# biscuitzb/COEB-SLAM

Measured on AMD Instinct MI355X. Metric: frames/sec ORB extract+match @640x480/1000 kp; 1/2/4/8 GPU + %HBM roofline, higher is better.
Workload: dtype u8; 1 GPU; 640x480, 8-level pyramid, 1000 kp, extract + Hamming match to prev frame (BASELINE configs[1]); width=640, height=480, nfeatures=1000, nlevels=8, halo_frames_per_rank=1, pipelines_per_gpu=3, streams_per_gpu=1, ranks=single, parallelism=frame-sharded x1 (no collectives), hw_queues=4, side_stream=own, side_stream_created=with the context

## Files before the change

coeb-slam_amd/csrc/coeb_extract.hip:

```cpp
#include <type_traits>
#include <cmath>
#include <hip/hip_runtime.h>

#include "coeb_internal.hpp"

namespace {

constexpr int kThreads = 256;
constexpr int kWaves = kThreads / 64;

__device__ __forceinline__ int lane_id() { return __lane_id(); }
__device__ __forceinline__ int wave_id() { return __builtin_amdgcn_readfirstlane(threadIdx.x >> 6); }
__device__ __forceinline__ void wave_sync_lds()
{
    __builtin_amdgcn_fence(__ATOMIC_RELEASE, "wavefront");
    __builtin_amdgcn_wave_barrier();
    __builtin_amdgcn_fence(__ATOMIC_ACQUIRE, "wavefront");
}
typedef unsigned int u32x4 __attribute__((ext_vector_type(4)));

__device__ __forceinline__ uint64_t lanemask_lt() { return (1ull << lane_id()) - 1ull; }

__device__ __forceinline__ int wave_sum(int v)
{
// ... 1565 lines not shown
            }
        } else {
            const int G = oct_team<NT>(nd, (K - (n - nd) + nd - 1) / nd);
            divide_nodes(G, S, nd, 0);
        }
        obar();
        int T = 0, nexp = 0;
        for (int base = 0; base < nd; base += NT) {
            const int j = base + tid;
            int e = 0, x = 0;
            if (j < nd) {
                const int4 q = s_cnt[j];
                e = (q.x > 0) + (q.y > 0) + (q.z > 0) + (q.w > 0);
                x = (q.x > 1) + (q.y > 1) + (q.z > 1) + (q.w > 1);
            }
            int tot, tot2;
            const int pre = block_scan_excl<NW>(e, &tot, sbuf);
            block_scan_excl<NW>(x, &tot2, sbuf);
            if (j < nd) s_base[j] = T + pre;
            T += tot;
            nexp += tot2;
        }
        obar();
        const int nnew = T + (n - nd);
        if (nnew > g.ncap) { if (tid == 0) atomicOr(b.err, 4); finish = true; break; }
        for (int j = tid; j < nd; j += NT) {
            const int k = s_work[j];
            const int4 q = s_cnt[j];
            const int s = S.start[k], bf = S.buf[k];
            const int4 r = S.rect[k];
            int a = s_base[j];
            int off = s;
            const int qq[4] = {q.x, q.y, q.z, q.w};
            for (int c4 = 0; c4 < 4; c4++) {
                if (qq[c4] > 0) {
                    const int pos = T - 1 - a;
                    int4 cr; int sx, sy;
                    child_rect(r, c4, &cr, &sx, &sy);
                    D.start[pos] = off; D.cnt[pos] = qq[c4]; D.alloc[pos] = alloc_ctr + a;
                    D.buf[pos] = bf ^ 1; D.rect[pos] = cr;
                    a++;
                }
                off += qq[c4];
            }
        }
        {
            int carry = 0;
            for (int base = 0; base < n; base += NT) {
                const int k = base + tid;
                const bool keep = k < n && S.cnt[k] <= 1;
                int tot;
                const int pre = block_scan_flag<NW>(keep, &tot, sbuf);
                if (keep) {
                    const int pos = T + carry + pre;
                    D.start[pos] = S.start[k]; D.cnt[pos] = S.cnt[k]; D.alloc[pos] = S.alloc[k];
                    D.buf[pos] = S.buf[k]; D.rect[pos] = S.rect[k];
                }
                carry += tot;
            }
        }
        obar();
        alloc_ctr += T;
        n = nnew;
        cs ^= 1;
        if (n >= N || n == prevSize) { finish = true; break; }
        if (n + nexp * 3 > N) { final_phase = true; break; }
    }

    while (final_phase && !finish) {
        const int prevSize = n;
        if (n > OCT_LMAX) { if (tid == 0) atomicOr(b.err, 4); break; }
        NodeRef S = nref(O, cs), D = nref(O, cs ^ 1);
        int m = 0;
        for (int base = 0; base < n; base += NT) {
            const int k = base + tid;
            const bool dv = k < n && S.cnt[k] > 1;
            int tot;
            const int pre = block_scan_flag<NW>(dv, &tot, sbuf);
            if (dv) s_work[m + pre] = k;
            m += tot;
        }
        for (int k = tid; k < n; k += NT) s_dead[k] = 0;
        obar();
        const int avg = m > 0 ? (K - (n - m) + m - 1) / m : 0;
        if (m > 0) divide_nodes(oct_team<NT>(m, avg), S, m, 1);
        for (int j = tid; j < m; j += NT) {
            const int k = s_work[j];
            s_push[j] = (int)(((uint32_t)S.cnt[k] << 16) | (uint32_t)S.alloc[k]);
        }
        obar();
        if (K < 32768 && alloc_ctr < 65536) {
            for (int j = tid; j < m; j += NT) {
                const int kj = s_push[j];
                int rank = 0;
#pragma unroll 8
                for (int i = 0; i < m; i++) rank += s_push[i] > kj;
                s_rank[j] = rank;
            }
        } else {
            for (int j = tid; j < m; j += NT) {
                const int k = s_work[j];
                const int cj = S.cnt[k], aj = S.alloc[k];
                int rank = 0;
                for (int i = 0; i < m; i++) {
                    const int ki = s_work[i];
                    const int ci = S.cnt[ki], ai = S.alloc[ki];
                    rank += (ci > cj) || (ci == cj && ai > aj);
                }
                s_rank[j] = rank;
            }
        }
        obar();
        for (int j = tid; j < m; j += NT) s_base[s_rank[j]] = j;
        obar();
        int nproc = m;
        {
            int carry = 0, found = 0x7fffffff;
            for (int base = 0; base < m; base += NT) {
                const int r = base + tid;
                int d = 0;
                if (r < m) {
                    const int4 q = s_cnt[s_base[r]];
                    d = (q.x > 0) + (q.y > 0) + (q.z > 0) + (q.w > 0) - 1;
                }
                int tot;
                const int pre = block_scan_excl<NW>(d, &tot, sbuf);
                if (r < m && n + carry + pre + d >= N) found = min(found, r);
                carry += tot;
            }
            int fr = found;
            for (int o = 32; o > 0; o >>= 1) fr = min(fr, __shfl_xor(fr, o, 64));
            if (lane == 0) sbuf[wv] = fr;
            obar();
            int mn = 0x7fffffff;
            for (int i = 0; i < NW; i++) mn = min(mn, sbuf[i]);
            obar();
            if (mn != 0x7fffffff) nproc = mn + 1;
        }
        int T = 0;
        for (int base = 0; base < nproc; base += NT) {
            const int r = base + tid;
            int e = 0;
            if (r < nproc) {
                const int4 q = s_cnt[s_base[r]];
                e = (q.x > 0) + (q.y > 0) + (q.z > 0) + (q.w > 0);
            }
            int tot;
            const int pre = block_scan_excl<NW>(e, &tot, sbuf);
            if (r < nproc) s_push[r] = T + pre;
            T += tot;
        }
        for (int j = tid; j < m; j += NT)
            if (s_rank[j] < nproc) s_dead[s_work[j]] = 1;
        obar();
        const int nnew = T + n - nproc;
        if (nnew > g.ncap) { if (tid == 0) atomicOr(b.err, 4); break; }
        divide_nodes(oct_team<NT>(nproc, avg), S, nproc, 2);
        for (int r = tid; r < nproc; r += NT) {
            const int j = s_base[r];
            const int k = s_work[j];
            const int s = S.start[k], bf = S.buf[k];
            const int4 pr = S.rect[k];
            const int4 qc = s_cnt[j];
            {
                int a = s_push[r];
                int off = s;
                const int qq[4] = {qc.x, qc.y, qc.z, qc.w};
                for (int c4 = 0; c4 < 4; c4++) {
                    if (qq[c4] > 0) {
                        const int pos = T - 1 - a;
                        int4 cr; int ssx, ssy;
                        child_rect(pr, c4, &cr, &ssx, &ssy);
                        D.start[pos] = off; D.cnt[pos] = qq[c4]; D.alloc[pos] = alloc_ctr + a;
                        D.buf[pos] = bf ^ 1; D.rect[pos] = cr;
                        a++;
                    }
                    off += qq[c4];
                }
            }
        }
        {
            int carry = 0;
            for (int base = 0; base < n; base += NT) {
                const int k = base + tid;
                const bool keep = k < n && !s_dead[k];
                int tot;
                const int pre = block_scan_flag<NW>(keep, &tot, sbuf);
                if (keep) {
                    const int pos = T + carry + pre;
                    D.start[pos] = S.start[k]; D.cnt[pos] = S.cnt[k]; D.alloc[pos] = S.alloc[k];
                    D.buf[pos] = S.buf[k]; D.rect[pos] = S.rect[k];
                }
                carry += tot;
            }
        }
        obar();
        alloc_ctr += T;
        n = nnew;
        cs ^= 1;
        if (n >= N || n == prevSize) finish = true;
    }
    if (COEB_OCT_CLOCK) oc_t2 = (long long)clock64();

    NodeRef S = nref(O, cs);
    uint32_t* out = b.lvl_kp + (int64_t)f * P->lvl_stride + g.out_off;
    const bool cull = !area && l < 8;
    const float scale = (l != 0) ? g.scale : 1.0f;
    int carry = 0;
    for (int base = 0; base < n; base += NT) {
        const int k = base + tid;
        uint32_t best = 0;
        bool keep = false;
        if (k < n) {
            const uint32_t* src = KB(S.buf[k]) + S.start[k];
            const int c = S.cnt[k];
            best = src[0];
            int maxr = key_s(best);
            for (int q = 1; q < c; q++) {
                const uint32_t kk = src[q];
                if (key_s(kk) > maxr) { best = kk; maxr = key_s(kk); }
            }
            const int x = key_x(best) + 16, y = key_y(best) + 16;
            best = pack_key(x, y, key_s(best));
            keep = !(cull && masked_out(dm, (float)x, (float)y, scale, P->W, P->H));
        }
        int tot;
        const int pre = block_scan_flag<NW>(keep, &tot, sbuf);
        if (keep) {
            if (carry + pre < g.out_cap) out[carry + pre] = best;
            else atomicOr(b.err, 8);
        }
        carry += tot;
    }
    if (tid == 0) b.lvl_n[(int64_t)f * P->L + l] = min(carry, g.out_cap);
    if (COEB_OCT_CLOCK && tid == 0) {
        const int wg = blockIdx.x + gridDim.x * blockIdx.y;
        if (wg < 4096) {
            long long* r = g_oct_clk + 6 * wg;
            r[0] = l; r[1] = K; r[2] = oc_w0;
            r[3] = (long long)clock64() - oc_t0; r[4] = oc_t1 - oc_t0; r[5] = oc_t2 - oc_t1;
        }
    }
}

__device__ float fast_atan2_dev(float y, float x)
{
    const float p1 = 0.9997878412794807f * (float)(180 / 3.1415926535897932384626433832795);
    const float p3 = -0.3258083974640975f * (float)(180 / 3.1415926535897932384626433832795);
    const float p5 = 0.1555786518463281f * (float)(180 / 3.1415926535897932384626433832795);
    const float p7 = -0.04432655554792128f * (float)(180 / 3.1415926535897932384626433832795);
    const float ax = fabsf(x), ay = fabsf(y);
    float a, c, c2;
    if (ax >= ay) {
        c = ay / (ax + (float)2.2204460492503131e-16);
        c2 = c * c;
        a = (((p7 * c2 + p5) * c2 + p3) * c2 + p1) * c;
    } else {
        c = ax / (ay + (float)2.2204460492503131e-16);
        c2 = c * c;
        a = 90.f - (((p7 * c2 + p5) * c2 + p3) * c2 + p1) * c;
    }
    if (x < 0) a = 180.f - a;
    if (y < 0) a = 360.f - a;
    return a;
}

__device__ void sincos_canon(float af, float* s, float* c)
{
    const double two_over_pi = 6.36619772367581382433e-01;
    const double pio2_1 = 1.57079632673412561417e+00;
    const double pio2_1t = 6.07710050650619224932e-11;
    const double S1 = -1.66666666666666324348e-01, S2 = 8.33333333332248946124e-03,
                 S3 = -1.98412698298579493134e-04, S4 = 2.75573137070700676789e-06,
                 S5 = -2.50507602534068634195e-08, S6 = 1.58969099521155010221e-10;
    const double C1 = 4.16666666666666019037e-02, C2 = -1.38888888888741095749e-03,
                 C3 = 2.48015872894767294178e-05, C4 = -2.75573143513906633035e-07,
                 C5 = 2.08757232129817482790e-09, C6 = -1.13596475577881948265e-11;
    const double x = (double)af;
    const double kd = rint(x * two_over_pi);
    double r = __builtin_fma(-kd, pio2_1, x);
    r = __builtin_fma(-kd, pio2_1t, r);
    const double z = r * r;
    const double v = z * r;
    const double sr = S2 + z * (S3 + z * (S4 + z * (S5 + z * S6)));
    const double sn = r + v * (S1 + z * sr);
    const double cr = z * (C1 + z * (C2 + z * (C3 + z * (C4 + z * (C5 + z * C6)))));
    const double hz = 0.5 * z;
    const double w = 1.0 - hz;
    const double cs = w + (((1.0 - w) - hz) + z * cr);
    const int q = ((int)kd) & 3;
    double so, co;
    if (q == 0) { so = sn; co = cs; }
    else if (q == 1) { so = cs; co = -sn; }
    else if (q == 2) { so = -sn; co = -cs; }
    else { so = -cs; co = sn; }
    *s = (float)so;
    *c = (float)co;
}

struct KeyPointOut { float x, y, size, angle, response; int octave, class_id; };

constexpr int kBlRow = 72, kBlRows = 37;
constexpr int kDescGroup = 2;
constexpr int kDescIcBatch = 32;
#ifndef COEB_DESC_KP
#define COEB_DESC_KP 8
#endif
template <int KP> constexpr int desc_slab() { return kBlRow * kBlRows * kDescGroup + 32 * KP; }
constexpr int kUmax[16] = {15, 15, 15, 15, 14, 14, 14, 13, 13, 12, 11, 10, 9, 8, 6, 3};

__device__ __forceinline__ uint32_t ic_mask(int av, int d)
{
    uint32_t w = 0;
    for (int i = 0; i < 4; i++) {
        const int u = 4 * d + i - 15;
        if (av < 16 && (u < 0 ? -u : u) <= kUmax[av]) w |= 0xFFu << (8 * i);
    }
    return w;
}

__device__ __forceinline__ uint32_t dpp_or_xor1(uint32_t v)
{
    return v | (uint32_t)__builtin_amdgcn_mov_dpp((int)v, 0xB1, 0xf, 0xf, false);
}
__device__ __forceinline__ uint32_t dpp_or_xor2(uint32_t v)
{
    return v | (uint32_t)__builtin_amdgcn_mov_dpp((int)v, 0x4E, 0xf, 0xf, false);
}
__device__ __forceinline__ uint32_t dpp_or_shl4(uint32_t v)
{
    return v | (uint32_t)__builtin_amdgcn_mov_dpp((int)v, 0x104, 0xf, 0xf, false);
}

template <bool kVec>
__device__ __forceinline__ void ic_row_load(const uint8_t* rp, uint4& c0, uint4& c1, uint4& c2)
{
    if (kVec) {
        c0 = reinterpret_cast<const uint4*>(rp)[0];
        c1 = reinterpret_cast<const uint4*>(rp)[1];
        c2 = reinterpret_cast<const uint4*>(rp)[2];
    } else {
        uint32_t q[12];
#pragma unroll
        for (int k = 0; k < 12; k++)
            q[k] = (uint32_t)rp[4 * k] | ((uint32_t)rp[4 * k + 1] << 8) | ((uint32_t)rp[4 * k + 2] << 16) |
                   ((uint32_t)rp[4 * k + 3] << 24);
        c0 = make_uint4(q[0], q[1], q[2], q[3]);
        c1 = make_uint4(q[4], q[5], q[6], q[7]);
        c2 = make_uint4(q[8], q[9], q[10], q[11]);
    }
}

template <bool kVec0, int KP>
__global__ __launch_bounds__(kThreads) void k_describe(const Plan* __restrict__ P, ExtractBufs b)
{
    constexpr int kLpk = 64 / KP;
    constexpr int kHl = kLpk / 2;
    constexpr int kNr = 16 / kHl;
    constexpr int kNb = kNr < 4 ? kNr : 4;
    static_assert(KP >= 2 && KP <= 32 && (KP & (KP - 1)) == 0, "KP: power of two in [2, 32]");
    __shared__ __attribute__((aligned(16))) uint8_t s_slab[kWaves][desc_slab<KP>()];
    __shared__ __attribute__((aligned(16))) uint32_t s_msk[17][8];
    if (threadIdx.x < 17 * 8) s_msk[threadIdx.x >> 3][threadIdx.x & 7] = ic_mask(threadIdx.x >> 3, threadIdx.x & 7);
    __syncthreads();
    const int2 bxy = block_xy();
    const int f = bxy.y;
    const int L = P->L;
    const int lane = lane_id(), wv = wave_id();
    const int nl = lane < L ? b.lvl_n[(int64_t)f * L + lane] : 0;
    int incl = nl;
    for (int o = 1; o < COEB_MAXL; o <<= 1) {
        const int y = __shfl_up(incl, o, 64);
        if (lane >= o) incl += y;
    }
    const int total = __builtin_amdgcn_readlane(incl, L - 1);
    if (bxy.x == 0 && threadIdx.x == 0) b.counts[f] = total;
    const int idx0 = (bxy.x * kWaves + wv) * KP;
    if (idx0 >= total) return;
    const int nk = min(KP, total - idx0);
    const int kq = lane / kLpk, half = (lane / kHl) & 1, qi = lane % kHl;
    const int id = idx0 + min(kq, nk - 1);
    int l = 0, start = 0;
    for (int q = 0; q < L - 1; q++) {
        const int e = __builtin_amdgcn_readlane(incl, q);
        if (id >= e) { l = q + 1; start = e; }
    }
    const LevelGeom& g = P->lv[l];
    const uint32_t key = b.lvl_kp[(int64_t)f * P->lvl_stride + g.out_off + (id - start)];
    const int x = key_x(key), y = key_y(key), sc = key_s(key);
    const uint8_t* img = level_ptr(P, b, f, l);
    uint32_t A = 0, S = 0;
    int m01 = 0;
    const int a = (x - 15) & 15;
    const uint32_t m8 = (a & 8) ? 0xFFFFFFFFu : 0u, m4 = (a & 4) ? 0xFFFFFFFFu : 0u;
    const uint8_t* rowp = img + (int64_t)y * g.pitch + (x - 15 - a);
    const int64_t spitch = half ? (int64_t)g.pitch : -(int64_t)g.pitch;
    const bool vec = kVec0 || l != 0;
    int aoff = 15;
    if (vec) {
        constexpr int kTasks = (93 + kLpk - 1) / kLpk;
        constexpr int kBatch = kDescIcBatch < kTasks ? kDescIcBatch : kTasks;
        constexpr uint64_t kUmaxPk = 0x3689ABCDDEEEFFFFull;
        const int j = lane % kLpk;
        const uint8_t* base0 = img + (int64_t)(y - 15) * g.pitch + (x - 15 - a);
#pragma unroll
        for (int i0 = 0; i0 < kTasks; i0 += kBatch) {
        uint4 cq[kBatch];
#pragma unroll
        for (int ii = 0; ii < kBatch; ii++) {
            const int i = i0 + ii;
            if (i >= kTasks) break;
            const int r = min(j + kLpk * i, 92);
            const int row = r / 3, ch = r - 3 * row;
            cq[ii] = *reinterpret_cast<const uint4*>(base0 + (int64_t)row * g.pitch + 16 * ch);
        }
#pragma unroll
        for (int ii = 0; ii < kBatch; ii++) {
            const int i = i0 + ii;
            if (i >= kTasks) break;
            const int r = j + kLpk * i;
            if (r < 93) {
                const int row = r / 3, ch = r - 3 * row;
                const int v = row - 15, av = v < 0 ? -v : v;
                const int um = (int)((kUmaxPk >> (4 * av)) & 15u);
                const uint32_t q[4] = {cq[ii].x, cq[ii].y, cq[ii].z, cq[ii].w};
                uint32_t rs = 0;
#pragma unroll
                for (int d = 0; d < 4; d++) {
                    const int u0 = 16 * ch + 4 * d - a - 15;
                    const int s0 = min(max(-um - u0, 0), 4), e0 = min(max(um - u0 + 1, 0), 4);
                    const uint32_t msk = (uint32_t)((1ull << (8 * e0)) - 1ull) & ~(uint32_t)((1ull << (8 * s0)) - 1ull);
                    const uint32_t pm = q[d] & msk;
                    A = __builtin_amdgcn_udot4(pm, (uint32_t)(u0 + 31) * 0x01010101u + 0x03020100u, A, false);
                    rs = __builtin_amdgcn_udot4(pm, 0x01010101u, rs, false);
                }
                S += rs;
                m01 += v * (int)rs;
            }
        }
        }
        aoff = 31;
    } else {
#pragma unroll
    for (int i0 = 0; i0 < kNr; i0 += kNb) {
        uint4 c[kNb][3];
#pragma unroll
        for (int r = 0; r < kNb; r++) {
            const uint8_t* rp = rowp + (qi + kHl * (i0 + r)) * spitch;
            if (vec) ic_row_load<true>(rp, c[r][0], c[r][1], c[r][2]);
            else ic_row_load<false>(rp, c[r][0], c[r][1], c[r][2]);
        }
#pragma unroll
        for (int r = 0; r < kNb; r++) {
            const int av = qi + kHl * (i0 + r);
            const uint32_t* msk = s_msk[(av == 0 && half) ? 16 : av];
            const uint32_t q[12] = {c[r][0].x, c[r][0].y, c[r][0].z, c[r][0].w, c[r][1].x, c[r][1].y,
                                    c[r][1].z, c[r][1].w, c[r][2].x, c[r][2].y, c[r][2].z, c[r][2].w};
            uint32_t r1[10], r2[9];
#pragma unroll
            for (int k = 0; k < 10; k++) r1[k] = (m8 & q[k + 2]) | (~m8 & q[k]);
#pragma unroll
            for (int k = 0; k < 9; k++) r2[k] = (m4 & r1[k + 1]) | (~m4 & r1[k]);
            uint32_t rs = 0;
#pragma unroll
            for (int d = 0; d < 8; d++) {
                const uint32_t pm = __builtin_amdgcn_alignbyte(r2[d + 1], r2[d], (uint32_t)(a & 3)) & msk[d];
                A = __builtin_amdgcn_udot4(pm, 0x03020100u + 0x04040404u * (uint32_t)d, A, false);
                rs = __builtin_amdgcn_udot4(pm, 0x01010101u, rs, false);
            }
            S += rs;
            m01 += av * (int)rs;
        }
    }
        if (half == 0) m01 = -m01;
    }
#pragma unroll
    for (int o = 1; o < kLpk; o <<= 1) {
        A += __shfl_xor(A, o, 64);
        S += __shfl_xor(S, o, 64);
        m01 += __shfl_xor(m01, o, 64);
    }
    const int m10 = (int)A - aoff * (int)S;
    const float angle = fast_atan2_dev((float)m01, (float)m10);
    const float factorPI = (float)(3.1415926535897932384626433832795 / 180.f);
    float bs, ac;
    sincos_canon(angle * factorPI, &bs, &ac);
    if (lane % kLpk == 0 && kq < nk) {
        float fx = (float)x, fy = (float)y;
        if (l != 0) { fx *= g.scale; fy *= g.scale; }
        KeyPointOut o;
        o.x = fx; o.y = fy; o.size = (float)g.size_i; o.angle = angle; o.response = (float)sc;
        o.octave = l; o.class_id = -1;
        reinterpret_cast<KeyPointOut*>(b.kps)[(int64_t)f * P->kcap + idx0 + kq] = o;
    }
    const int4 pa = reinterpret_cast<const int4*>(b.pattern)[lane];
    float px0[4], py0[4], px1[4], py1[4];
#pragma unroll
    for (int t = 0; t < 4; t++) {
        const int pw = t == 0 ? pa.x : t == 1 ? pa.y : t == 2 ? pa.z : pa.w;
        px0[t] = (float)(int8_t)(pw & 0xff); py0[t] = (float)(int8_t)((pw >> 8) & 0xff);
        px1[t] = (float)(int8_t)((pw >> 16) & 0xff); py1[t] = (float)(int8_t)(pw >> 24);
    }
    uint8_t* slab = s_slab[wv];
    uint32_t* dsl = reinterpret_cast<uint32_t*>(slab + kBlRow * kBlRows * kDescGroup);
    const int xoff = x - ((x - 18) & ~15);
    const uint8_t* blur_f = b.blur + (int64_t)f * P->blur_stride;
    static_assert(kDescGroup == 2, "staging below is written for 2 patches per step");
    uint4 qa0, qa1, qa2, qb0, qb1, qb2;
    const int ty0 = (y - 18) >> 3, dy = (y - 18) & 7, tymax = ((y + 18) >> 3) - ty0;
    const int porg = (int)g.blur_off + (int)blur_tile_off((x - 18) & ~15, ty0 * 8, g.bpitch);
    const int trs = g.bpitch * 8;
    const int lo = ((lane >> 3) & 3) * 128 + (lane & 7) * 16;
    const int tr0 = lane >> 5;
#define COEB_LOAD_PATCH(t, q0, q1, q2)                                                          \
    {                                                                                           \
        const int tt_ = min((t), nk - 1);                                                       \
        const uint8_t* o_ = blur_f + __builtin_amdgcn_readlane(porg, tt_ * kLpk) + lo;          \
        const int trs_ = __builtin_amdgcn_readlane(trs, tt_ * kLpk);                            \
        const int tm_ = __builtin_amdgcn_readlane(tymax, tt_ * kLpk);                           \
        q0 = *reinterpret_cast<const uint4*>(o_ + min(tr0, tm_) * trs_);                        \
        q1 = *reinterpret_cast<const uint4*>(o_ + min(tr0 + 2, tm_) * trs_);                    \
        q2 = *reinterpret_cast<const uint4*>(o_ + min(tr0 + 4, tm_) * trs_);                    \
    }
    COEB_LOAD_PATCH(0, qa0, qa1, qa2)
    COEB_LOAD_PATCH(1, qb0, qb1, qb2)
    for (int t0 = 0; t0 < nk; t0 += kDescGroup) {
        {
            auto put = [&](uint8_t* base, int row, int c, uint4 v) {
                uint2* d = reinterpret_cast<uint2*>(base + row * kBlRow + 16 * c);
                d[0] = make_uint2(v.x, v.y);
                d[1] = make_uint2(v.z, v.w);
            };
            uint8_t* pb = slab + kBlRow * kBlRows;
            const int dya = __builtin_amdgcn_readlane(dy, min(t0, nk - 1) * kLpk);
            const int dyb = __builtin_amdgcn_readlane(dy, min(t0 + 1, nk - 1) * kLpk);
            const int c = (lane >> 3) & 3, r = 8 * tr0 + (lane & 7);
            auto put_t = [&](uint8_t* base, int row, uint4 v) {
                if ((unsigned)row < (unsigned)kBlRows) put(base, row, c, v);
            };
            put_t(slab, r - dya, qa0);
            put_t(slab, r + 16 - dya, qa1);
            put_t(slab, r + 32 - dya, qa2);
            put_t(pb, r - dyb, qb0);
            put_t(pb, r + 16 - dyb, qb1);
            put_t(pb, r + 32 - dyb, qb2);
        }
        wave_sync_lds();
        if (t0 + kDescGroup < nk) {
            COEB_LOAD_PATCH(t0 + 2, qa0, qa1, qa2)
            COEB_LOAD_PATCH(t0 + 3, qb0, qb1, qb2)
        }
#pragma unroll
        for (int k = 0; k < kDescGroup; k++) {
            const int t = t0 + k;
            if (t >= nk) break;
            const float tb = __int_as_float(__builtin_amdgcn_readlane(__float_as_int(bs), t * kLpk));
            const float ta = __int_as_float(__builtin_amdgcn_readlane(__float_as_int(ac), t * kLpk));
            const uint8_t* bc = slab + k * kBlRow * kBlRows + 18 * kBlRow + __builtin_amdgcn_readlane(xoff, t * kLpk);
            const f32x2 AB = {ta, tb}, BA = {tb, ta};
            uint32_t nib = 0;
#pragma unroll
            for (int tt = 0; tt < 4; tt++) {
                const f32x2 t0 = f32x2{py0[tt], py0[tt]} * AB, t1 = f32x2{py1[tt], py1[tt]} * AB;
                const f32x2 rc0 = __builtin_elementwise_fma(f32x2{px0[tt], px0[tt]}, BA, f32x2{t0.x, -t0.y});
                const f32x2 rc1 = __builtin_elementwise_fma(f32x2{px1[tt], px1[tt]}, BA, f32x2{t1.x, -t1.y});
                const int o0 = (int)__builtin_fmaf(rintf(rc0.x), (float)kBlRow, rintf(rc0.y));
                const int o1 = (int)__builtin_fmaf(rintf(rc1.x), (float)kBlRow, rintf(rc1.y));
                nib |= (uint32_t)(bc[o0] < bc[o1]) << tt;
            }
            uint32_t dw = nib << (4 * (lane & 7));
            dw = dpp_or_shl4(dpp_or_xor2(dpp_or_xor1(dw)));
            if ((lane & 7) == 0) dsl[8 * t + (lane >> 3)] = dw;
        }
        wave_sync_lds();
    }
#undef COEB_LOAD_PATCH
    uint4* gd = reinterpret_cast<uint4*>(b.desc + ((int64_t)f * P->kcap + idx0) * 32);
    if (lane < 2 * nk) gd[lane] = reinterpret_cast<const uint4*>(dsl)[lane];
}

}

int fast_timing_read(unsigned long long* out)
{
    static unsigned long long h[256 * 8];
    if (hipMemcpyFromSymbol(h, HIP_SYMBOL(g_fast_clk), sizeof(h)) != hipSuccess) return -1;
    for (int k = 0; k < 8; k++) {
        out[k] = 0;
        for (int i = 0; i < 256; i++) out[k] += h[i * 8 + k];
    }
    static const unsigned long long z[256 * 8] = {};
    return hipMemcpyToSymbol(HIP_SYMBOL(g_fast_clk), z, sizeof(z)) == hipSuccess ? 0 : -1;
}

int oct_timing_read(long long* out)
{
    return hipMemcpyFromSymbol(out, HIP_SYMBOL(g_oct_clk), sizeof(long long) * 4096 * 6) == hipSuccess ? 0 : -1;
}

int launch_extract(const Plan& plan, const Plan* d_plan, const ExtractBufs& b, int F, hipStream_t s,
                   ProfileHook* prof, const SideStream* side)
{
    prof_begin(prof, "k_dynmask", s);
    hipLaunchKernelGGL(k_dynmask, dim3((F + 63) / 64), dim3(64), 0, s, b, F, plan.W, plan.H);
    prof_end(prof, s);
    BlurWork bw;
    bw.L = plan.L;
    int items = 0;
    const int brows = 32;
    static_assert(brows % 8 == 0, "bands start on tile rows");
    bw.brows = brows;
    for (int l = 0; l < plan.L; l++) {
        const LevelGeom& g = plan.lv[l];
        bw.nstrips[l] = (g.w + kBlurCols - 1) / kBlurCols;
        bw.item_off[l] = items;
        bw.nquads[l] = (bw.nstrips[l] + 3) / 4;
        bw.bh[l] = 0;
        items += bw.nquads[l] * ((g.h + brows - 1) / brows);
    }
    bw.item_off[plan.L] = items;
    const char* pb = coeb_switch("COEB_PYR_BYTES");
    const bool pyr_bytes = pb && atoi(pb) != 0;
    const char* frb = coeb_switch("COEB_FAST_RB");
    const int fast_rbytes = frb && atoi(frb) == kFastRowBytes ? kFastRowBytes : fast_rb(plan);
    const int fast_lds = kWaves * fast_wave_lds(plan, fast_rbytes);
    constexpr int kFastPerBlock = kWaves;
    auto blur = [&](hipStream_t st, int i0, int i1) {
        if (i1 <= i0) return;
        BlurWork w = bw;
        w.item0 = i0; w.item1 = i1;
        prof_begin(prof, "k_blur", st);
        hipLaunchKernelGGL(k_blur_rows, dim3((i1 - i0 + kWaves - 1) / kWaves, F), dim3(kThreads), 0,
                           st, d_plan, b, w);
        prof_end(prof, st);
    };
    auto fast = [&](hipStream_t st, int l0, int l1) {
        l1 = std::min(l1, plan.L);
        if (l1 <= l0) return;
        prof_begin(prof, "k_fast", st);
        const int c0 = plan.lv[l0].cell0, c1 = l1 < plan.L ? plan.lv[l1].cell0 : plan.ncells;
        hipLaunchKernelGGL(fast_rbytes == kFastRowBytesM ? k_fast<kFastRowBytesM> : k_fast<kFastRowBytes>,
                           dim3((c1 - c0 + kFastPerBlock - 1) / kFastPerBlock, F), dim3(kThreads), fast_lds,
                           st, d_plan, b, b.cells, c0, c1);
        prof_end(prof, st);
    };
    const bool split = side && side->s && plan.L > 1;
    const int m = split ? 2 : 0;
    if (split) {
        (void)hipEventRecord(side->fork, s);
        (void)hipStreamWaitEvent(side->s, side->fork, 0);
        blur(side->s, 0, bw.item_off[1]);
        fast(side->s, 0, 1);
    }
    for (int l = 1; l < plan.L; l++) {
        const LevelGeom& g = plan.lv[l];
        const LevelGeom& gp = plan.lv[l - 1];
        const uint8_t* src = l == 1 ? b.gray : b.pyr + gp.pyr_off;
        const int64_t src_fs = l == 1 ? (int64_t)plan.W * plan.H : plan.pyr_stride;
        prof_begin(prof, "k_pyr_level", s);
        const bool rows = g.rows_ok && ((gp.pitch | (int)(src_fs & 3) | (int)((uintptr_t)src & 3)) & 3) == 0;
        if (rows && !pyr_bytes) {
            hipLaunchKernelGGL(k_pyr_rows, dim3((g.w + PR_COLS - 1) / PR_COLS, (g.h + kWaves * PR_ROWS - 1) / (kWaves * PR_ROWS), F),
                               dim3(kThreads), 0, s, src, src_fs, gp.pitch, gp.h, b.pyr + g.pyr_off, plan.pyr_stride,
                               g.pitch, g.w, g.h, b.rtab + g.rtab_off, g.xmax, resize_simd_end(g.w),
                               reinterpret_cast<const int4*>(b.rtab + g.yrow_off), b.rtab + g.band_off);
        } else {
            int tsw, tsh;
            pyr_tile_lds(gp.w, gp.h, g.w, g.h, &tsw, &tsh);
            hipLaunchKernelGGL(k_pyr_level, dim3((g.w + PT_W - 1) / PT_W, (g.h + PT_H - 1) / PT_H, F), dim3(kThreads),
                               tsw * tsh, s, src, src_fs, gp.pitch, gp.w, gp.h, b.pyr + g.pyr_off, plan.pyr_stride,
                               g.pitch, g.w, g.h, b.rtab + g.rtab_off, g.xmax, resize_simd_end(g.w), tsw, tsh);
        }
        prof_end(prof, s);
        if (split && l == m - 1) {
            (void)hipEventRecord(side->mid, s);
            (void)hipStreamWaitEvent(side->s, side->mid, 0);
            blur(side->s, bw.item_off[1], bw.item_off[m]);
            fast(side->s, 1, m);
        }
    }
    constexpr int kOctThreads = 256;
    int oct_kl, oct_lds;
    oct_launch_keys(plan, F, &oct_kl, &oct_lds);
    lds_limit_max((const void*)k_octree<kOctThreads>);
    auto octree = [&](hipStream_t st, int l0, int l1) {
        if (l1 <= l0) return;
        prof_begin(prof, "k_octree", st);
        hipLaunchKernelGGL(k_octree<kOctThreads>, dim3(F, l1 - l0), dim3(kOctThreads), oct_lds, st, d_plan, b, l0, plan.oct_w,
                           oct_kl);
        prof_end(prof, st);
    };
    if (split) {
        (void)hipEventRecord(side->pyr_done, s);
        (void)hipStreamWaitEvent(side->s, side->pyr_done, 0);
        blur(side->s, bw.item_off[m], items);
        (void)hipEventRecord(side->join, side->s);
    } else {
        blur(s, 0, items);
    }
    fast(s, m, plan.L);
    if (split) (void)hipStreamWaitEvent(s, side->join, 0);
    octree(s, 0, plan.L);
    prof_begin(prof, "k_describe", s);
    const bool vec0 = plan.W % 16 == 0 && (reinterpret_cast<uintptr_t>(b.gray) & 15) == 0;
    constexpr int KP = COEB_DESC_KP;
    if (vec0)
        hipLaunchKernelGGL((k_describe<true, KP>), dim3((plan.kcap + kWaves * KP - 1) / (kWaves * KP), F), dim3(kThreads), 0,
                           s, d_plan, b);
    else
        hipLaunchKernelGGL((k_describe<false, KP>), dim3((plan.kcap + kWaves * KP - 1) / (kWaves * KP), F), dim3(kThreads), 0,
                           s, d_plan, b);
    prof_end(prof, s);
    return hipGetLastError() == hipSuccess ? 0 : -1;
}
```

Before: 390,800 frames/s.

## Rewrite ORB intensity-centroid path with branchless circle masks and strided row pointers

Reworks the vectorized intensity-centroid moment loop. Instead of computing per-dword min/max byte masks for every row, it precomputes packed umax words at compile time and builds the circular-window mask via byte-wise add/bitop3 tricks, so each dword needs one mask plus two dot4 ops. Row addresses are advanced by a fixed stride per task, and all loads are issued before any compute. It also makes the patch-to-LDS stores branchless by sending out-of-range rows to a dummy LDS area, and skips the LDS mask table init and barrier in the vec-only variant. The cost is more LDS per wave, KP restricted to 8 or 16, and more registers held by the full load batch.

```diff
diff --git a/coeb-slam_amd/csrc/coeb_extract.hip b/coeb-slam_amd/csrc/coeb_extract.hip
--- a/coeb-slam_amd/csrc/coeb_extract.hip
+++ b/coeb-slam_amd/csrc/coeb_extract.hip
@@ -1891,11 +1891,11 @@
 
 constexpr int kBlRow = 72, kBlRows = 37;
 constexpr int kDescGroup = 2;
-constexpr int kDescIcBatch = 32;
+constexpr int kDescDummy = 80;
 #ifndef COEB_DESC_KP
 #define COEB_DESC_KP 8
 #endif
-template <int KP> constexpr int desc_slab() { return kBlRow * kBlRows * kDescGroup + 32 * KP; }
+template <int KP> constexpr int desc_slab() { return kBlRow * kBlRows * kDescGroup + 32 * KP + kDescDummy; }
 constexpr int kUmax[16] = {15, 15, 15, 15, 14, 14, 14, 13, 13, 12, 11, 10, 9, 8, 6, 3};
 
 __device__ __forceinline__ uint32_t ic_mask(int av, int d)
@@ -1907,6 +1907,19 @@
     }
     return w;
 }
+
+template <int kStep, int kN>
+struct IcUmWords {
+    uint32_t w[kN];
+    constexpr IcUmWords() : w{}
+    {
+        for (int m = 0; m < kN; m++)
+            for (int i = 0; i < 8; i++) {
+                const int row = kStep * m + i, v = row - 15;
+                if (row <= 30) w[m] |= (uint32_t)kUmax[v < 0 ? -v : v] << (4 * i);
+            }
+    }
+};
 
 __device__ __forceinline__ uint32_t dpp_or_xor1(uint32_t v)
 {
@@ -1947,11 +1960,13 @@
     constexpr int kHl = kLpk / 2;
     constexpr int kNr = 16 / kHl;
     constexpr int kNb = kNr < 4 ? kNr : 4;
-    static_assert(KP >= 2 && KP <= 32 && (KP & (KP - 1)) == 0, "KP: power of two in [2, 32]");
+    static_assert(KP == 8 || KP == 16, "KP: 8 or 16");
     __shared__ __attribute__((aligned(16))) uint8_t s_slab[kWaves][desc_slab<KP>()];
-    __shared__ __attribute__((aligned(16))) uint32_t s_msk[17][8];
-    if (threadIdx.x < 17 * 8) s_msk[threadIdx.x >> 3][threadIdx.x & 7] = ic_mask(threadIdx.x >> 3, threadIdx.x & 7);
-    __syncthreads();
+    __shared__ __attribute__((aligned(16))) uint32_t s_msk[kVec0 ? 1 : 17][8];
+    if constexpr (!kVec0) {
+        if (threadIdx.x < 17 * 8) s_msk[threadIdx.x >> 3][threadIdx.x & 7] = ic_mask(threadIdx.x >> 3, threadIdx.x & 7);
+        __syncthreads();
+    }
     const int2 bxy = block_xy();
     const int f = bxy.y;
     const int L = P->L;
@@ -1988,45 +2003,46 @@
     int aoff = 15;
     if (vec) {
         constexpr int kTasks = (93 + kLpk - 1) / kLpk;
-        constexpr int kBatch = kDescIcBatch < kTasks ? kDescIcBatch : kTasks;
-        constexpr uint64_t kUmaxPk = 0x3689ABCDDEEEFFFFull;
+        constexpr IcUmWords<kLpk, (kTasks + 2) / 3> kUm;
+        constexpr uint32_t hb = 0x80808080u;
         const int j = lane % kLpk;
-        const uint8_t* base0 = img + (int64_t)(y - 15) * g.pitch + (x - 15 - a);
-#pragma unroll
-        for (int i0 = 0; i0 < kTasks; i0 += kBatch) {
-        uint4 cq[kBatch];
-#pragma unroll
-        for (int ii = 0; ii < kBatch; ii++) {
-            const int i = i0 + ii;
-            if (i >= kTasks) break;
-            const int r = min(j + kLpk * i, 92);
+        const uint8_t* base0 = img + ((y - 15) * g.pitch + (x - 15 - a));
+        const int64_t step = kLpk * g.pitch;
+        const uint8_t* pk[3];
+        uint32_t Wk[3];
+        int vk[3];
+#pragma unroll
+        for (int k = 0; k < 3; k++) {
+            const int r = j + kLpk * k;
             const int row = r / 3, ch = r - 3 * row;
-            cq[ii] = *reinterpret_cast<const uint4*>(base0 + (int64_t)row * g.pitch + 16 * ch);
-        }
-#pragma unroll
-        for (int ii = 0; ii < kBatch; ii++) {
-            const int i = i0 + ii;
-            if (i >= kTasks) break;
-            const int r = j + kLpk * i;
-            if (r < 93) {
-                const int row = r / 3, ch = r - 3 * row;
-                const int v = row - 15, av = v < 0 ? -v : v;
-                const int um = (int)((kUmaxPk >> (4 * av)) & 15u);
-                const uint32_t q[4] = {cq[ii].x, cq[ii].y, cq[ii].z, cq[ii].w};
-                uint32_t rs = 0;
-#pragma unroll
-                for (int d = 0; d < 4; d++) {
-                    const int u0 = 16 * ch + 4 * d - a - 15;
-                    const int s0 = min(max(-um - u0, 0), 4), e0 = min(max(um - u0 + 1, 0), 4);
-                    const uint32_t msk = (uint32_t)((1ull << (8 * e0)) - 1ull) & ~(uint32_t)((1ull << (8 * s0)) - 1ull);
-                    const uint32_t pm = q[d] & msk;
-                    A = __builtin_amdgcn_udot4(pm, (uint32_t)(u0 + 31) * 0x01010101u + 0x03020100u, A, false);
-                    rs = __builtin_amdgcn_udot4(pm, 0x01010101u, rs, false);
-                }
-                S += rs;
-                m01 += v * (int)rs;
-            }
-        }
+            pk[k] = base0 + (row * g.pitch + 16 * ch);
+            Wk[k] = (uint32_t)(16 * ch - a + 16) * 0x01010101u + 0x03020100u;
+            vk[k] = row - 15;
+        }
+        uint4 cq[kTasks];
+#pragma unroll
+        for (int i = 0; i < kTasks; i++) {
+            if (kLpk * i + kLpk - 1 < 93 || j + kLpk * i < 93) pk[i % 3] += i < 3 ? 0 : step;
+            cq[i] = *reinterpret_cast<const uint4*>(pk[i % 3]);
+        }
+#pragma unroll
+        for (int i = 0; i < kTasks; i++) {
+            const int k = i % 3, m = i / 3;
+            const bool ok = kLpk * i + kLpk - 1 < 93 || j + kLpk * i < 93;
+            const uint32_t um = (kUm.w[m] >> (4 * (vk[k] + 15))) & 15u;
+            const uint32_t c_lo = ok ? __builtin_amdgcn_perm(0u, um + 97u, 0u) : 0u;
+            const uint32_t c_hi = 0xC1C1C1C1u - c_lo;
+            const uint32_t q[4] = {cq[i].x, cq[i].y, cq[i].z, cq[i].w};
+            uint32_t rs = 0;
+#pragma unroll
+            for (int d = 0; d < 4; d++) {
+                const uint32_t W = Wk[k] + 0x04040404u * (uint32_t)d;
+                const uint32_t in = (uint32_t)__builtin_amdgcn_bitop3_b32(W + c_lo, W + c_hi, hb, 0x20) >> 7;
+                rs = __builtin_amdgcn_udot4(q[d], in, rs, false);
+                A = __builtin_amdgcn_udot4(q[d], W & ((hb - in) | hb), A, false);
+            }
+            S += rs;
+            m01 += __mul24(vk[k] + kLpk * m, (int)rs);
         }
         aoff = 31;
     } else {
@@ -2124,8 +2140,10 @@
             const int dya = __builtin_amdgcn_readlane(dy, min(t0, nk - 1) * kLpk);
             const int dyb = __builtin_amdgcn_readlane(dy, min(t0 + 1, nk - 1) * kLpk);
             const int c = (lane >> 3) & 3, r = 8 * tr0 + (lane & 7);
+            uint8_t* dmy = slab + kBlRow * kBlRows * kDescGroup + 32 * KP;
             auto put_t = [&](uint8_t* base, int row, uint4 v) {
-                if ((unsigned)row < (unsigned)kBlRows) put(base, row, c, v);
+                const bool in = (unsigned)row < (unsigned)kBlRows;
+                put(in ? base : dmy, in ? row : 0, c, v);
             };
             put_t(slab, r - dya, qa0);
             put_t(slab, r + 16 - dya, qa1);
```

After: 393,300 frames/s (median of 6 runs). About the same (+0.6%).
